# pacificclimate/VIC

Measured on AMD Instinct MI355X. Metric: cell-timesteps/s, higher is better.
Workload: dtype f64

## Files before the change

vic_amd/csrc/vic_ctx.hpp:

```cpp
#pragma once
#include <cstddef>
#include <type_traits>
#include "vic_step.hpp"

using namespace vic;

constexpr int HS_STATE = 3, HS_CLS_SHIFT = 2;

constexpr int EBC_W_POST = offsetof(SurfEBConst, delta_t) / 8, EBC_W_ALWAYS = offsetof(SurfEBConst, ice0) / 8,
              EBC_W_FROZEN = offsetof(SurfEBConst, kappa_snow) / 8, EBC_W_SNOWCOV = offsetof(SurfEBConst, LongSnowIn) / 8,
              EBC_W_INCL = offsetof(SurfEBConst, lmoist) / 8, EBC_W_EVAP = offsetof(SurfEBConst, Wdew) / 8,
              EBC_W_CANOPY = offsetof(SurfEBConst, Cs2) / 8;
constexpr int EBM_W_FEED = offsetof(SurfEBMut, deltaCC) / 8, EBM_W_IN3 = offsetof(SurfEBMut, Tsnow_surf) / 8,
              EBM_W_TSNOW = offsetof(SurfEBMut, ra_used) / 8, EBM_W_RA1 = EBM_W_TSNOW + 1, EBM_W_VV = offsetof(SurfEBMut, vv) / 8,
              EBM_W_KEEP = offsetof(SurfEBMut, Tnew2) / 8;
static_assert(offsetof(SurfEBMut, fusion) / 8 == EBM_W_IN3 - 1 && offsetof(SurfEBMut, layerevap) / 8 == EBM_W_VV + 3, "SurfEBMut layout");
constexpr size_t CW_SV = sizeof(SurfSolve) / 8, CW_EBM = sizeof(SurfEBMut) / 8, CW_EBC = EBC_W_CANOPY,
                 CW_P = sizeof(SubStep) / 8, CW_L = sizeof(SubLoop) / 8, CW_C = sizeof(StepConst) / 8;
constexpr size_t CO_SV = 0, CO_EBM = CO_SV + CW_SV, CO_EBC = CO_EBM + CW_EBM, CO_P = CO_EBC + CW_EBC, CO_L = CO_P + CW_P,
                 CO_C = CO_L + CW_L, CO_W = CO_C + CW_C;
constexpr size_t CW_W = sizeof(WCarry) / 8, CO_WM = CO_W + CW_W;
template <int NN> constexpr size_t ctx_words() { return CO_WM + sizeof(WCarryMulti<NN>) / 8; }
static_assert(sizeof(StepConstPost) <= sizeof(StepConst), "StepConstPost is parked in StepConst's words");
constexpr size_t CW_L_HEAD = offsetof(SubLoop, st_AlbedoOver) / 8;
constexpr size_t CW_SV_ITER = offsetof(SurfSolve, Tsurf) / 8;

constexpr int CTX_GROUP = 8, CTX_GROUP_B = 2;
constexpr size_t CTX_NA = sizeof(SurfSolve) / 8 + sizeof(SurfEBMut) / 8 + offsetof(SurfEBConst, Cs2) / 8;
static_assert(CTX_NA == CO_P, "region A of the context slab = what the evaluation kernel reads");
constexpr int CTXR_ITER = 0, CTXR_COMMON = 16, CTXR_CLASS = 48, CTXR_SNOW = 64, CTXR_COLD = 72, CTXR_END = 104;
struct CtxMap { unsigned char slab[CTX_NA]; int end[6]; };
constexpr int ctx_map_run(CtxMap& m, int at, size_t first, size_t last) {
  for (size_t w = first; w < last; w++) m.slab[w] = (unsigned char)at++;
  return at;
}
constexpr CtxMap ctx_make_map() {
  CtxMap m{};
  int at = ctx_map_run(m, CTXR_ITER, CO_SV, CO_SV + CW_SV_ITER);
  m.end[0] = at;
  at = ctx_map_run(m, CTXR_COMMON, CO_EBM + EBM_W_FEED, CO_EBM + EBM_W_TSNOW);
  at = ctx_map_run(m, at, CO_EBM + EBM_W_RA1, CO_EBM + EBM_W_RA1 + 1);
  at = ctx_map_run(m, at, CO_EBC, CO_EBC + EBC_W_ALWAYS);
  m.end[1] = at;
  at = ctx_map_run(m, CTXR_CLASS, CO_EBC + EBC_W_ALWAYS, CO_EBC + EBC_W_FROZEN);
  at = ctx_map_run(m, at, CO_EBC + EBC_W_INCL, CO_EBC + EBC_W_CANOPY);
  m.end[2] = at;
  at = ctx_map_run(m, CTXR_SNOW, CO_EBC + EBC_W_FROZEN, CO_EBC + EBC_W_INCL);
  m.end[3] = at;
// ... 1 lines not shown
  m.end[4] = at;
  at = ctx_map_run(m, at, CO_EBM + EBM_W_TSNOW, CO_EBM + EBM_W_TSNOW + 1);
  at = ctx_map_run(m, at, CO_EBM, CO_EBM + EBM_W_FEED);
  at = ctx_map_run(m, at, CO_EBM + EBM_W_VV, CO_EBM + CW_EBM);
  m.end[5] = at;
  return m;
}
constexpr CtxMap CTX_MAP = ctx_make_map();
constexpr bool ctx_map_is_permutation() {
  bool used[CTXR_END] = {};
  for (size_t w = 0; w < CTX_NA; w++) {
    if (CTX_MAP.slab[w] >= CTXR_END || used[CTX_MAP.slab[w]]) return false;
    used[CTX_MAP.slab[w]] = true;
  }
  int n = 0;
  for (int i = 0; i < CTXR_END; i++) n += used[i] ? 1 : 0;
  return n == (int)CTX_NA;
}
static_assert(ctx_map_is_permutation(), "parking map of region A");
static_assert(CTXR_ITER % CTX_GROUP == 0 && CTXR_COMMON % CTX_GROUP == 0 && CTXR_CLASS % CTX_GROUP == 0 && CTXR_SNOW % CTX_GROUP == 0
              && CTXR_COLD % CTX_GROUP == 0 && CTXR_END % CTX_GROUP == 0, "every range of the parking map starts on a sector boundary");
static_assert(CTX_MAP.end[0] == CTXR_COMMON && CTX_MAP.end[1] <= CTXR_CLASS && CTX_MAP.end[2] <= CTXR_SNOW && CTX_MAP.end[3] <= CTXR_COLD
              && CTX_MAP.end[4] <= CTXR_COLD + CTX_GROUP && CTX_MAP.end[5] <= CTXR_END && CTXR_END - CTX_MAP.end[5] < CTX_GROUP,
              "ranges of the parking map; the tail of SurfSolve, which every evaluation fetches, in one sector");
static_assert(CTX_MAP.end[1] - CTXR_COMMON == 31 && CTX_MAP.end[2] - CTXR_CLASS == 13,
              "the iteration's inputs: 4 sectors for every class, 2 more for frozen soil / evaporation / canopy");
constexpr size_t CTX_NA_PAD = CTXR_END;
constexpr size_t ctx_padded_words(size_t words) {
  return CTX_NA_PAD + ((words > CTX_NA ? words - CTX_NA : 0) + CTX_GROUP_B - 1) / CTX_GROUP_B * CTX_GROUP_B;
}
struct CtxRef {
  unsigned long long* p;
  int lane;
  VIC_DEV static CtxRef at(unsigned long long* base, size_t words_per_hru, size_t g) {
    return CtxRef{base + (g >> 6) * (ctx_padded_words(words_per_hru) * 64), (int)(g & 63)};
  }
  VIC_DEV unsigned long long* word(size_t W) const {
    if (W < CTX_NA) {
      const size_t S = CTX_MAP.slab[W];
      return p + (S / CTX_GROUP) * (64 * CTX_GROUP) + lane * CTX_GROUP + (S % CTX_GROUP);
    }
    const size_t V = W - CTX_NA;
    return p + CTX_NA_PAD * 64 + (V / CTX_GROUP_B) * (64 * CTX_GROUP_B) + lane * CTX_GROUP_B + (V % CTX_GROUP_B);
  }
};
template <class T>
VIC_DEV void ctx_put(const CtxRef& r, size_t word0, const T& v) {
// ... 5 lines not shown
  for (int i = 0; i < NW; i++) *r.word(word0 + i) = tmp[i];
}
template <class T>
VIC_DEV void ctx_get(const CtxRef& r, size_t word0, T& v) {
  static_assert(sizeof(T) % 8 == 0 && std::is_trivially_copyable<T>::value, "context structs are arrays of 8-byte words");
  constexpr int NW = sizeof(T) / 8;
  unsigned long long tmp[NW];
#pragma unroll
  for (int i = 0; i < NW; i++) tmp[i] = *r.word(word0 + i);
  __builtin_memcpy(&v, tmp, sizeof(T));
}

template <class T>
VIC_DEV void ctx_put_words(const CtxRef& r, size_t word0, const T& v, int first, int last) {
  constexpr int NW = sizeof(T) / 8;
#pragma unroll
  for (int i = 0; i < NW; i++)
    if (i >= first && i < last) {
      unsigned long long w;
      __builtin_memcpy(&w, reinterpret_cast<const char*>(&v) + 8 * i, 8);
      *r.word(word0 + i) = w;
    }
}
template <class T>
VIC_DEV void ctx_get_words(const CtxRef& r, size_t word0, T& v, int first, int last) {
  constexpr int NW = sizeof(T) / 8;
#pragma unroll
  for (int i = 0; i < NW; i++)
    if (i >= first && i < last) {
      const unsigned long long w = *r.word(word0 + i);
      __builtin_memcpy(reinterpret_cast<char*>(&v) + 8 * i, &w, 8);
    }
}

VIC_DEV int surf_eb_class(const SurfEBConst& c) {
  return (c.frozen_on ? EBG_FROZEN : 0) | ((c.snow_coverage > 0 && !c.INCLUDE_SNOW) ? EBG_SNOWCOV : 0) | (c.INCLUDE_SNOW ? EBG_INCL : 0)
         | (!c.SNOWING ? EBG_EVAP : 0) | ((c.VEG && !c.SNOWING) ? EBG_CANOPY : 0);
}
VIC_DEV void ebc_put(const CtxRef& cx, const SurfEBConst& c, int cls) {
  ctx_put_words(cx, CO_EBC, c, 0, EBC_W_ALWAYS);
  if (cls & EBG_FROZEN) ctx_put_words(cx, CO_EBC, c, EBC_W_ALWAYS, EBC_W_FROZEN);
  if (cls & EBG_SNOWCOV) ctx_put_words(cx, CO_EBC, c, EBC_W_FROZEN, EBC_W_SNOWCOV);
  if (cls & EBG_INCL) ctx_put_words(cx, CO_EBC, c, EBC_W_SNOWCOV, EBC_W_INCL);
  if (cls & EBG_EVAP) ctx_put_words(cx, CO_EBC, c, EBC_W_INCL, EBC_W_EVAP);
  if (cls & EBG_CANOPY) ctx_put_words(cx, CO_EBC, c, EBC_W_EVAP, EBC_W_CANOPY);
}
// ... 9 lines not shown
```

vic_amd/csrc/vic_implicit.hpp:

```cpp
#pragma once
#include "vic_profile.hpp"

namespace vic {

enum { PI_MOIST = 0, PI_ICE, PI_KAPPA, PI_CS, PIMP };

struct IArgs {
  int ncell, nhru, Nband;
  const double* pimp;
  const int* hpi;
  const double* cell_params;
  const int* hkey;
  int* fb_list;
  int* fb_count;
  int* lastexp;
  int* cursor;
};

struct ImplicitSolver {
  static constexpr int M = VIC_MID_NODES + 2;
  int n, NOFLUX, EXP_TRANS;
  double deltat, Bexp, Ts, Tb;
  double T0[M], moist[M], ice[M], kappa[M], Cs[M];
  double ice_new[M], Cs_new[M], kappa_new[M];
// ... 180 lines not shown
          const double Dp = cv.s(CP_DP);
          S.Bexp = a.EXP_TRANS ? (a.NOFLUX ? log(Dp + 1.) / (double)S.n : log(Dp + 1.) / (double)(S.n + 1)) : 0.0;
          S.Ts = S.T0[0];
          S.Tb = a.NOFLUX ? S.T0[S.n] : S.T0[S.n + 1];
          for (int q = 0; q < ImplicitSolver::M; q++) xs[q] = 0;
          S.begin(xs);
          k = 0;
          have = true;
        }
      }
    }
    if (!__any(have)) break;
    bool failed = false;
    if (have) {
      const bool conv = S.trial(xs, k);
      k++;
      if (conv) {
        const int ps = a.pslot[hru];
        double* __restrict__ rec = a.pout + (size_t)hru * pout_hru_stride(Nn) + ps * pout_stride(Nn);
        const int le = x.lastexp[hru];
        unsigned long long meta = 1ull << 32;
        if (le >= 0) {
          const double* __restrict__ src = a.pout + (size_t)hru * pout_hru_stride(Nn) + le * pout_stride(Nn);
          meta = (unsigned long long)__double_as_longlong(src[Nn]) | (1ull << 32);
          if (le != ps)
            for (int q = 0; q < (Nn + 1) / 2; q++) rec[Nn + 1 + q] = src[Nn + 1 + q];
        } else {
          int* __restrict__ cnt = reinterpret_cast<int*>(rec + Nn + 1);
          for (int q = 0; q < Nn; q++) cnt[q] = 0;
        }
        rec[0] = S.T0[0];
        for (int q = 0; q < S.n; q++) rec[q + 1] = xs[q];
        if (!a.NOFLUX) rec[Nn - 1] = S.T0[Nn - 1];
        rec[Nn] = __longlong_as_double((long long)meta);
        a.pout[(size_t)hru * pout_hru_stride(Nn) + pout_key(Nn, ps)] = S.T0[0];
        if (le >= 0) x.lastexp[hru] = ps;
        have = false;
      } else if (k >= ImplicitSolver::MAXTRIAL) {
        failed = true;
        x.lastexp[hru] = a.pslot[hru];
        have = false;
      }
    }
    list_append(x.fb_list, x.fb_count, a.cap, failed, failed ? x.hkey[hru] : 0, hru);
  }
}
```

vic_amd/csrc/vic_kernels.hpp:

```cpp
#pragma once
#include <cstddef>
#include "vic_glacier.hpp"
#include "vic_profile.hpp"
#include "vic_implicit.hpp"
#include "vic_ctx.hpp"
#include "vic_hru_io.hpp"

using namespace vic;

template <int NN, bool GLAC>
VIC_DEV int hru_prologue(const KArgs& a, int g, const HruId& id, const CellView& cv, const VegLib& vl, const Forcing& fc, const Soil3& s3,
                         HruWork<NN>& w, StepConst& C, bool node_props = true) {
  const Opt& o = a.o;
  const size_t nh = a.nhru;
  const int month = a.dmy.month;
  const int veg_idx = id.veg_idx;
  int err = 0;
  C.veg_idx = veg_idx; C.band = id.band; C.is_art_bare = id.is_art_bare ? 1 : 0;
#pragma unroll
  for (int l = 0; l < 3; l++) C.root[l] = (double)(float)a.hpd[(size_t)(HPD_ROOT0 + l) * nh + g];
  if (o.BLOWING) {
    C.sigma_slope = (double)(float)a.hpd[(size_t)HPD_SIGMA_SLOPE * nh + g]; C.lag_one = (double)(float)a.hpd[(size_t)HPD_LAG_ONE * nh + g];
    C.fetch = (double)(float)a.hpd[(size_t)HPD_FETCH * nh + g];
  } else { C.sigma_slope = 0; C.lag_one = 0; C.fetch = 0; }
// ... 179 lines not shown
    load_untouched_state<NN>(a, g, w);
    if constexpr (MULTI) {
      ctx_get(cx, CO_C, C);
      WCarryMulti<NN> km;
      ctx_get(cx, CO_WM, km);
      carry_in_multi<NN>(km, w);
    } else {
      StepConstPost q;
      ctx_get(cx, CO_C, q);
      step_const_post_in(q, P.UnderStory, C);
      C.veg_idx = id.veg_idx; C.band = id.band; C.is_art_bare = id.is_art_bare ? 1 : 0;
      C.overstory = (vl.f(id.veg_idx, VL_OVERSTORY) != 0.0) ? 1 : 0;
#pragma unroll
      for (int l = 0; l < 3; l++) C.root[l] = (double)(float)a.hpd[(size_t)(HPD_ROOT0 + l) * a.nhru + g];
    }
    {
      WCarry k;
      ctx_get(cx, CO_W, k);
      carry_in<NN>(k, w);
    }
    PROF_ADD(11, t_stage);
    PROF_T0(t_post);
    const double* __restrict__ po = a.pout + (size_t)g * pout_hru_stride(Nn) + sv.final_slot * pout_stride(Nn);
    const int* __restrict__ poc = reinterpret_cast<const int*>(po + Nn + 1);
    double Tprof[NN];
    int cntprof[NN];
    const unsigned long long flags = (unsigned long long)__double_as_longlong(po[Nn]);
#pragma unroll
    for (int n = 0; n < NN; n++) {
      Tprof[n] = (n < Nn) ? po[n] : 0.0;
      cntprof[n] = (n < Nn) ? poc[n] : 0;
    }
    using mask_t = typename NodeBound<NN>::mask_t;
    sf_sub_post<NN>(o, cv, vl, s3, fc, a.dmy, C, w, L, P, eb, sv, Tprof, cntprof,
                    (mask_t)(flags & ((1ull << NodeBound<NN>::ok_bit) - 1ull)));
    PROF_ADD(12, t_post);
    more = true;
  }
  bool pend = false;
  int key = 0;
  if ((FIRST || MULTI) && more && L.hidx < L.endhidx) {
    if constexpr (FIRST || MULTI) {
      SubStep P;
      SurfEB eb;
      SurfSolve sv;
      PROF_T0(t_pre);
      sf_sub_pre<NN>(o, cv, vl, s3, fc, a.dmy, C, w, L, P, eb, sv);
      PROF_ADD(13, t_pre);
      PROF_T0(t_put);
      ctx_put(cx, CO_SV, sv);
      ctx_put_words(cx, CO_EBM, static_cast<const SurfEBMut&>(eb), 0, EBM_W_KEEP);
      const int cls = surf_eb_class(eb);
      ebc_put(cx, eb, cls);
// ... 33 lines not shown
      if (o.IMPLICIT) {
        double* __restrict__ im = a.pimp + (size_t)g * Nn * PIMP;
#pragma unroll
        for (int n = 0; n < NN; n++)
          if (n < Nn) {
            im[n * PIMP + PI_MOIST] = w.nd.moist[n]; im[n * PIMP + PI_ICE] = (n == 0) ? eb.delta_t : w.nd.ice[n];
            im[n * PIMP + PI_KAPPA] = w.nd.kappa[n]; im[n * PIMP + PI_CS] = w.nd.Cs[n];
          }
        a.lastexp[g] = -1;
      }
      a.ts[g] = sv.x;
      a.pslot[g] = 0;
      if (o.QUICK_SOLVE) {
        int tmpNnodes = 0;
#pragma unroll
        for (int n = NN - 1; n >= 0; n--)
          if (n <= Nn - 5 && w.nd.T[n] >= 0 && w.nd.T[(n + 1 < NN) ? n + 1 : n] < 0) tmpNnodes = n + 1;
        if (tmpNnodes == 0) tmpNnodes = (w.nd.T[0] <= 0 && w.nd.T[1] >= 0) ? Nn : 3;
        else tmpNnodes += 4;
        a.jl[g] = (sv.stage == SurfSolve::ROOT_QUICK) ? tmpNnodes - 1 : (o.NOFLUX ? Nn : Nn - 1);
      }
      a.pout[(size_t)g * pout_hru_stride(Nn) + pout_key(Nn, 0)] = NAN;
      a.pout[(size_t)g * pout_hru_stride(Nn) + pout_key(Nn, 1)] = NAN;
      a.hstate[g] = 1 | (cls << HS_CLS_SHIFT);
      pend = true;
      PROF_ADD(14, t_put);
    }
  } else {
    PROF_T0(t_end);
    if (more && !sf_end<NN>(o, cv, s3, C, w, L)) err |= VICGPU_CELLERR_SOLVER;
    PROF_ADD(15, t_end);
    hru_epilogue<NN>(a, g, cv, s3, C, w, err, false);
    a.hstate[g] = 0;
  }
  list_append(a.list, a.count, a.list_cap, pend, key, g);
  PROF_ADD(0, t_stage);
  PROF_WAVE(0);
  PROF_LANE(1);
}

struct EArgs {
  Opt o;
  LaunchMap map;
  int ncell, nhru, Nn;
  const int* glist;
  int gcount;
  const double* cell_params;
// ... 6 lines not shown
  int* jl;
  int* hstate;
  int* list_next;
  int* count_next;
  int list_cap;
  const int* hkey;
  int* profile_next;
  int* pend_list_next;
  int* pend_count_next;
  int pend_cap;
  int list_thr;
  const int* pend_list_cur;
  const int* pend_prefix;
  const int* npend_cur;
  int implicit;
  const double* veglib;
  const double* forcing;
  const int* fcol;
  int ncol;
  int month;
};

constexpr int EVAL_WAVES = 2;
__global__ __launch_bounds__(64) VIC_WAVES_PER_EU(EVAL_WAVES, EVAL_WAVES) void vic_surf_eval(const EArgs a) {
  if (blockIdx.x == 0 && threadIdx.x == 0) *a.profile_next = 0;
  const int npend = *a.npend_cur;
  int g;
  if (npend <= a.list_thr) {
    if ((int)blockIdx.x * 64 >= npend) return;
    __shared__ int prefix[PEND_STRIPES + 1];
    for (int b = threadIdx.x; b < PEND_STRIPES + 1; b += 64) prefix[b] = a.pend_prefix[b];
    __syncthreads();
    const int gi = blockIdx.x * 64 + threadIdx.x;
    if (gi >= npend) return;
    int lo = 0, hi = PEND_STRIPES;
#pragma unroll
    for (int it = 0; it < 6; it++) {
      const int mid = (lo + hi) >> 1;
      const bool up = prefix[mid] <= gi;
      lo = up ? mid : lo; hi = up ? hi : mid;
    }
    g = a.pend_list_cur[(size_t)lo * a.pend_cap + (gi - prefix[lo])];
  } else {
    const int gi = a.map.index(blockIdx.x, threadIdx.x, a.gcount);
    if (gi < 0) return;
    g = a.glist ? a.glist[gi] : gi;
  }
  const int hs = a.hstate[g];
  if ((hs & HS_STATE) != 1) return;
  const int cls = hs >> HS_CLS_SHIFT;
  const size_t nh = a.nhru;
  const int c = a.hpi[(size_t)HPI_CELL * nh + g];
  const int veg_idx = a.hpi[(size_t)HPI_VEG_INDEX * nh + g];
  const int ps = a.pslot[g];
  CellView cv{a.cell_params, a.ncell, c, a.o.Nnode, a.o.Nband};
  const Soil3 s3 = load_soil3(cv);
  SurfSolve sv;
  SurfEB eb;
  const CtxRef cx = CtxRef::at(a.ctx, a.ctx_words, g);
  ctx_get(cx, CO_SV, sv);
  ebc_get(cx, eb, cls);
  const bool is_final = sv.stage == SurfSolve::FINAL;
  const int slot = sv.on_record ? sv.final_slot : ps;
  {
    SurfEBMut& m = eb;
    if (is_final) ctx_get_words(cx, CO_EBM, m, 0, EBM_W_KEEP);
    else {
      if (cls & EBG_INCL) ctx_get_words(cx, CO_EBM, m, 0, EBM_W_FEED);
      ctx_get_words(cx, CO_EBM, m, EBM_W_FEED, EBM_W_IN3);
      if (cls & EBG_SNOWCOV) ctx_get_words(cx, CO_EBM, m, EBM_W_IN3, EBM_W_TSNOW);
      if (cls & EBG_CANOPY) ctx_get_words(cx, CO_EBM, m, EBM_W_RA1, EBM_W_RA1 + 1);
    }
  }
  {
    const VegLib vl{a.veglib};
    const Forcing fc{a.forcing, nullptr, a.ncell, c, a.o.NR + 1, a.fcol[g], a.ncol};
    surf_cell_fill(eb, cv, vl, s3, fc, eb.hidx, veg_idx, a.month);
  }
  const double* __restrict__ rec = a.pout + (size_t)g * pout_hru_stride(a.Nn);
  const double* __restrict__ po = rec + slot * pout_stride(a.Nn);
  const bool ok = (((unsigned long long)__double_as_longlong(po[a.Nn])) >> record_ok_bit(node_bound(a.Nn))) & 1ull;
  if (sv.stage == SurfSolve::FINAL) sv.final_slot = slot;
  const double fx = ok ? eb.eval(a.o, s3, sv.x, po[1], po[2]) : ERROR_VAL;
  const bool was_quick = sv.stage == SurfSolve::ROOT_QUICK;
  const int stage_before = sv.stage;
  const double x_eval = sv.x;
  surf_solve_consume(a.o, sv, eb, eb, fx);
  bool at_root = false;
  if (stage_before == SurfSolve::ROOT && sv.stage == SurfSolve::FINAL && !a.implicit && !a.o.QUICK_SOLVE && !(cls & EBG_INCL) && sv.ok
      && sv.fbflag == 0 && sv.Tsurf == x_eval && fabs(fx) < 1.e30) {
    sv.final_slot = slot;
    surf_solve_consume(a.o, sv, eb, eb, fx);
    at_root = true;
  }
  if (was_quick && sv.stage != SurfSolve::ROOT_QUICK) {
    a.jl[g] = (sv.stage == SurfSolve::ROOT && a.o.NOFLUX) ? a.Nn : a.Nn - 1;
    a.pout[(size_t)g * pout_hru_stride(a.Nn) + pout_key(a.Nn, 0)] = NAN;
    a.pout[(size_t)g * pout_hru_stride(a.Nn) + pout_key(a.Nn, 1)] = NAN;
  }
  bool need_solve = sv.stage != SurfSolve::DONE;
  if (sv.stage == SurfSolve::FINAL && !a.implicit) {
    if (rec[pout_key(a.Nn, slot)] == sv.x) { sv.final_slot = slot; sv.on_record = 1; need_solve = false; }
    else if (rec[pout_key(a.Nn, slot ^ 1)] == sv.x) { sv.final_slot = slot ^ 1; sv.on_record = 1; need_solve = false; }
  }
  if (sv.stage == stage_before && (sv.stage == SurfSolve::ROOT || sv.stage == SurfSolve::ROOT_QUICK)) ctx_put_words(cx, CO_SV, sv, 0, (int)CW_SV_ITER);
  else ctx_put(cx, CO_SV, sv);
  if (sv.stage == SurfSolve::DONE) {
    const SurfEBMut& m = eb;
    if (at_root) {
      ctx_put_words(cx, CO_EBM, m, EBM_W_KEEP, (int)CW_EBM);
      ctx_put_words(cx, CO_EBM, m, EBM_W_TSNOW, EBM_W_TSNOW + 1);
      if (cls & EBG_FROZEN) ctx_put_words(cx, CO_EBM, m, EBM_W_IN3 - 1, EBM_W_IN3);
      if (cls & EBG_CANOPY) ctx_put_words(cx, CO_EBM, m, EBM_W_VV, EBM_W_VV + 6);
      else if (cls & EBG_EVAP) ctx_put_words(cx, CO_EBM, m, EBM_W_VV + 3, EBM_W_VV + 4);
    } else ctx_put(cx, CO_EBM, m);
  } else if (cls & EBG_INCL) ctx_put_words(cx, CO_EBM, static_cast<const SurfEBMut&>(eb), 0, EBM_W_FEED);
  if (sv.stage == SurfSolve::DONE) a.hstate[g] = 2;
  else if (need_solve) { a.ts[g] = sv.x; a.pslot[g] = slot ^ 1; }
  list_append(a.list_next, a.count_next, a.list_cap, need_solve, a.hkey[g], g);
  {
    const bool pend = sv.stage != SurfSolve::DONE;
    const unsigned long long m = __ballot(pend);
    if (m != 0) {
      const int lane = (int)__lane_id(), lead = __ffsll((long long)m) - 1, stripe = blockIdx.x % PEND_STRIPES;
      int base = 0;
      if (lane == lead) base = atomicAdd(a.pend_count_next + stripe * PEND_CNT_STRIDE, __popcll(m));
      base = __shfl(base, lead);
      if (pend) a.pend_list_next[(size_t)stripe * a.pend_cap + base + __popcll(m & ((1ull << lane) - 1ull))] = g;
    }
// ... 3 lines not shown
```

vic_amd/csrc/vic_pipeline.hpp:

```cpp
#pragma once
#include <hip/hip_runtime.h>
#include <stdio.h>
#include <stdlib.h>
#include <string.h>
#include <algorithm>
#include <chrono>
#include <condition_variable>
#include <memory>
#include <mutex>
#include <string>
#include <vector>
#include "vicgpu.h"
#include "vic_profile.hpp"
#include "vic_putdata.hpp"
#include "vic_host.hpp"
#include "vic_implicit.hpp"
#include "vic_ctx.hpp"
#include "vic_hru_io.hpp"
#include "vic_kernels.hpp"
#include "vic_aux_kernels.hpp"
#include "vic_records.hpp"
#include "vic_copy_cells.hpp"
#include "vic_params.hpp"
#include "vic_state_update.hpp"
// ... 52 lines not shown
  DevBuf<int> d_hstate, d_pslot, d_hkey, d_lastexp, d_jl;
  DevBuf<double> d_pimp;
  std::vector<FdChunk> chunks;
  bool put_on = false;
  int out_nrow = 0;
  OutLayout out_lay;
  DevBuf<double> d_out_data, d_out_agg, d_pb;
  DevBuf<unsigned char> d_rowagg;
};

constexpr int COPY_NKEY = 4;
constexpr int COPY_KEY_ROWS[COPY_NKEY] = {HPI_BAND, HPI_VEG_CLASS, HPI_IS_GLACIER, HPI_IS_ARTIFICIAL_BARE};

struct Tuning {
  bool node_newton = false;
  int eval_list_pct = 75;
  int nchunk = 1;
  int profile_waves_pct = 100;
  bool xcd_map = true;
  bool trace_rounds = false;
  bool trace = false;
  bool stats = false;
  int copy_stage_mb = 256;
};
static Tuning read_tuning(int node_solver, int ncell) {
  Tuning t;
  t.node_newton = node_solver == VIC_NODE_SOLVER_NEWTON;
  if (const char* ev = getenv("VICGPU_NODE_SOLVER")) t.node_newton = (strcmp(ev, "newton") == 0);
  if (const char* ev = getenv("VICGPU_EVAL_LIST_PCT")) {
    const int pct = atoi(ev);
    if (pct >= 0 && pct <= 100) t.eval_list_pct = pct;
  }
  t.nchunk = (ncell >= 20000) ? 2 : 1;
  if (const char* ev = getenv("VICGPU_CHUNKS")) t.nchunk = atoi(ev);
  if (t.nchunk < 1) t.nchunk = 1;
  if (t.nchunk > 16) t.nchunk = 16;
  if (t.nchunk > ncell) t.nchunk = ncell;
  t.profile_waves_pct = t.nchunk > 1 ? 50 : 100;
  if (const char* ev = getenv("VICGPU_PROFILE_WAVES_PCT")) {
    const int pct = atoi(ev);
    if (pct >= 5 && pct <= 100) t.profile_waves_pct = pct;
  }
  t.xcd_map = getenv("VICGPU_NO_XCD_MAP") == nullptr;
  t.trace_rounds = getenv("VICGPU_TRACE_ROUNDS") != nullptr;
  t.trace = getenv("VICGPU_TRACE") != nullptr;
  t.stats = getenv("VICGPU_STATS") != nullptr;
  if (const char* ev = getenv("VICGPU_COPY_STAGE_MB")) {
    const int mb = atoi(ev);
    if (mb >= 0 && mb <= 65536) t.copy_stage_mb = mb;
  }
  return t;
}


struct RecordsJoin {
  std::mutex m;
  std::condition_variable cv;
  std::vector<int> arrived;
  int queued = 0;
  int status = 0;
  std::string err;
  void start(int nrecords) { arrived.assign(nrecords, 0); queued = 0; status = 0; err.clear(); }
  bool arrive(int k, int nlane) { std::lock_guard<std::mutex> lk(m); return ++arrived[k] == nlane; }
  void join_queued(int k) { { std::lock_guard<std::mutex> lk(m); queued = k + 1; } cv.notify_all(); }
  int wait_queued(int k, std::string* why) {
    std::unique_lock<std::mutex> lk(m);
    cv.wait(lk, [&]() { return queued > k || status != 0; });
    if (status != 0) *why = err;
    return status;
  }
  void fail(int st, const std::string& why) {
    { std::lock_guard<std::mutex> lk(m); if (status == 0) { status = st; err = why; } }
    cv.notify_all();
// ... 251 lines not shown
  const int nsub = c->o.NF;
  for (int p = 1; p <= nsub; p++) {
    int nmax = ch->gcount;
    int npend = -1;
    int rb_list[RB_DEPTH];
    int rb_first = -1;
    for (int round = 0;; round++) {
      pa.list = ch->d_list[cur]; pa.count = cnt_list(ch->d_count, cur); pa.count_zero = cnt_list(ch->d_count, cur ^ 1);
      pa.pend_counts = cnt_list(ch->d_count, cur); pa.pend_stripes = cnt_stripes(ch->d_count, cur);
      pa.pend_stripes_zero = cnt_stripes(ch->d_count, cur ^ 1);
      if (c->o.IMPLICIT) {
        HIPCHK(ch, hipMemsetAsync(ch->d_fb_count, 0, sizeof(int) * (NBUCKET + 1), st));
        const int nblk = std::min(std::max((nmax + 63) / 64, 1), 4096);
        hipLaunchKernelGGL(vic_profile_solve_implicit, dim3(nblk), dim3(64), 0, st, pa, ia);
        HIPCHK(ch, hipGetLastError());
        pa.list = ch->d_fb_list; pa.count = ch->d_fb_count;
      }
      HIPCHK(ch, NODE_DISPATCH(Nn, launch_profile, pa, nmax, c->profile_waves, c->tune.node_newton, st));
      ea.list_next = ch->d_list[cur ^ 1]; ea.count_next = cnt_list(ch->d_count, cur ^ 1);
      ea.pend_list_next = ch->d_plist[cur ^ 1]; ea.pend_count_next = cnt_stripes(ch->d_count, cur ^ 1);
      ea.pend_list_cur = ch->d_plist[cur];
      ea.list_thr = round > 0 ? list_thr : -1;
      const bool sparse = npend >= 0 && npend <= ea.list_thr;
      hipLaunchKernelGGL(vic_surf_eval, dim3(sparse ? ((npend + 63) / 64 > 0 ? (npend + 63) / 64 : 1) : ea.map.nblocks(ch->gcount)), dim3(64), 0, st, ea);
      HIPCHK(ch, hipGetLastError());
      cur ^= 1;
      ch->rounds++;
      if (c->tune.trace_rounds) {
        int n = 0, np = 0;
        if (fd_read_count(ch, cur, &n, &np) != VICGPU_OK) return VICGPU_ERR_HIP;
        fprintf(stderr, "vicgpu rounds: chunk %d sub-step %d round %d leaves %d solves + %d evaluation-only of %d\n", (int)(ch - &c->dom.chunks[0]), p, round, n, np - n, ch->gcount);
      }
      if (round + 2 >= FREE_ROUNDS) {
        const int slot = round % RB_DEPTH;
        if (rb_first < 0) rb_first = round;
        HIPCHK(ch, hipMemcpyAsync(ch->h_count + slot * CNT_TOTAL, ch->d_count, sizeof(int) * CNT_TOTAL, hipMemcpyDeviceToHost, st));
        HIPCHK(ch, hipEventRecord(ch->readback[slot], st));
        rb_list[slot] = cur;
      }
      if (rb_first >= 0 && round - RB_LAG >= rb_first) {
        const int slot = (round - RB_LAG) % RB_DEPTH;
        HIPCHK(ch, hipEventSynchronize(ch->readback[slot]));
        const int* h = ch->h_count + slot * CNT_TOTAL;
        int n = 0;
        for (int b = 0; b < NBUCKET; b++) n += h[rb_list[slot] * CNT_LIST_STRIDE + b];
        const int np = cnt_pending(h, rb_list[slot]);
        if (np == 0) break;
// ... 307 lines not shown
```

vic_amd/csrc/vic_profile.hpp:

```cpp
#pragma once
#include "vic_surface.hpp"

namespace vic {

constexpr int NBUCKET = 2 * (VIC_MID_NODES + 2);
static_assert(NBUCKET <= 64, "one lane per work-list segment when the pending total is summed");
constexpr int PEND_STRIPES = 64, PEND_CNT_STRIDE = 32;

VIC_DEV void list_append(int* __restrict__ list, int* count, int cap, bool pred, int key, int g) {
  if (__ballot(pred) == 0) return;
  unsigned long long mine = 0;
#pragma unroll 1
  for (int k = 0; k < NBUCKET; k++) {
    const unsigned long long m = __ballot(pred && key == k);
    if (key == k) mine = m;
  }
  const int lane = (int)__lane_id();
  const int rank = __popcll(mine & ((1ull << lane) - 1ull));
  int base = 0;
  if (pred && rank == 0) base = atomicAdd(count + key, __popcll(mine));
  base = __shfl(base, pred ? __ffsll((long long)mine) - 1 : lane);
  if (pred) list[(size_t)key * cap + base + rank] = g;
}

struct PArgs {
  const double* __restrict__ pin;
  const double* __restrict__ ts;
  double* __restrict__ pout;
  const int* __restrict__ pslot;
  const int* __restrict__ list;
  const int* __restrict__ count;
  int cap;
  int* next;
  int* count_zero;
  const int* pend_counts;
  const int* pend_stripes;
  int* pend_stripes_zero;
  int* pend_prefix;
  int* pend_out;
  int Nn, NOFLUX, EXP_TRANS, TFALLBACK;
  const int* jl;
};

__host__ __device__ inline int pout_stride(int Nn) { return Nn + 1 + (Nn + 1) / 2; }
__host__ __device__ inline int pout_hru_stride(int Nn) { return 2 * pout_stride(Nn) + 2; }
__host__ __device__ inline int pout_key(int Nn, int slot) { return 2 * pout_stride(Nn) + slot; }

constexpr int LOCKSTEP_GATE = 16;

constexpr double NODE_ROOT_RANGE = SOIL_DT + Brent::MAXTRIES * Brent::TSTEP;
constexpr double NODE_NEWTON_TOL = 1.e-8;
constexpr double NODE_PREDICT_TOL2 = 1.e-7;
constexpr int NODE_PREDICT_MAXIT = 12;
constexpr double NODE_NEWTON_ACCEPT = 2.e-11;
constexpr int NODE_NEWTON_MAXIT = 200;

struct NodeK {
  double AT0, B, C, D, EI, S, G, Y, EM, EMM;
  VIC_DEV void load(const double* __restrict__ r) {
    AT0 = r[PR_AT0]; B = r[PR_B]; C = r[PR_C]; D = r[PR_D]; EI = r[PR_EI]; S = r[PR_S]; G = r[PR_G]; Y = r[PR_Y];
    EM = r[PR_EMOIST]; EMM = r[PR_EMM];
  }
  VIC_DEV double eice(double T, double& Eu, bool& curved) const {
    Eu = G * exp(Y * ln_pos(-T));
    curved = true;
    if (Eu > EMM) { Eu = EMM; curved = false; }
    double Ei = EM - Eu;
    if (Ei < 0.) { Ei = 0.; curved = false; }
    if (Ei > EMM) { Ei = EMM; curved = false; }
// ... 262 lines not shown
      PROF_WAVE(16); PROF_VOTE(17, sweeping);
#pragma unroll
      for (int j = 1; j < NN; j++) {
        if (j < jlast) {
          const double oldT = T[j];
          const double Tdn = (j == Nn - 1) ? oldT : T[(j + 1 < NN) ? j + 1 : j], Tup = T[j - 1];
          const double T0j = T0(j);
          NodeK Kj;
          if (j == NN - 1) Kj.load(a.pin + ((size_t)hru * Nn + j) * PREC);
          else {
            constexpr int q = 0;
            const int jj = (j < NN - 1) ? j : 1 + q;
            Kj.AT0 = kAT0[jj]; Kj.B = kB[jj]; Kj.C = kC[jj]; Kj.D = kD[jj]; Kj.EI = kEI[jj]; Kj.S = kS[jj]; Kj.EMM = kEMM[jj];
            Kj.G = KL(0, jj); Kj.Y = KL(1, jj); Kj.EM = KL(2, jj);
          }
          bool failed;
          double newT;
          const bool swj = sweeping && j < jl_lane;
          if (j == 1) newT = node_visit<true, NEWTON>(swj, frozen_on, EXP_TRANS, Kj, oldT, Tdn, Tup, T0j, failed);
          else newT = node_visit<false, NEWTON>(swj, frozen_on, EXP_TRANS, Kj, oldT, Tdn, Tup, T0j, failed);
          if (swj) {
            if (failed) {
              if (a.TFALLBACK) {
                int* cnt = reinterpret_cast<int*>(a.pout + (size_t)hru * pout_hru_stride(Nn) + ps * pout_stride(Nn) + Nn + 1);
                if (evcnt == 0) {
#pragma unroll
                  for (int k = 0; k < NN; k++) cnt[k] = 0;
                }
                evcnt = 1;
                cnt[j] += 1;
                newT = T0j; fbmask |= (1u << j);
              } else { ok = false; sweeping = false; }
            }
            if (sweeping) {
              T[j] = newT;
              const double diff = fabs(oldT - newT);
              if (diff > maxdiff) maxdiff = diff;
            }
          }
        }
      }
      if (sweeping) {
        if (maxdiff <= threshold) { converged = true; sweeping = false; }
        else if (it >= MAXIT) sweeping = false;
        else it++;
      }
    }
    PROF_ADD(21, t_sweep);
    PROF_T0(t_fin);
    if (have && !sweeping) {
      double T0v[NN];
      int cadd[NN];
#pragma unroll
      for (int k = 0; k < NN; k++) T0v[k] = T0(k);
      profile_finish<NN>(a.jl ? (jl_lane + 1 < Nn ? jl_lane + 1 : Nn) : Nn, a.TFALLBACK != 0, converged, ok, fbmask, T, T0v, cadd);
      double* __restrict__ rec = a.pout + (size_t)hru * pout_hru_stride(Nn) + ps * pout_stride(Nn);
      int* __restrict__ cnt = reinterpret_cast<int*>(rec + Nn + 1);
#pragma unroll
      for (int k = 0; k < NN; k++) rec[k] = T[k];
      rec[Nn] = __longlong_as_double((long long)((unsigned long long)fbmask | ((unsigned long long)(ok ? 1 : 0) << 32)));
#pragma unroll
      for (int k = 0; k < NN; k++) {
        if (evcnt == 0) cnt[k] = cadd[k];
        else cnt[k] += cadd[k];
      }
      a.pout[(size_t)hru * pout_hru_stride(Nn) + pout_key(Nn, ps)] = T0(0);
      have = false;
    }
    PROF_ADD(24, t_fin);
  }
#undef T0
#undef KL
}

constexpr int LS_WAVES = 2;
template <int NN, bool NEWTON>
__global__ __launch_bounds__(64) VIC_WAVES_PER_EU(LS_WAVES, LS_WAVES) void vic_profile_solve_lockstep(const PArgs a) {
  using mask_t = typename NodeBound<NN>::mask_t;
  constexpr bool T0_LDS = NN <= VIC_MID_NODES;
  __shared__ int bcount[NBUCKET];
  __shared__ double Tl[NN * 64];
  __shared__ double T0l[T0_LDS ? NN * 64 : 1];
  const int lane = threadIdx.x;
#define T(j) Tl[(j) * 64 + lane]
#define T0(j) (T0_LDS ? T0l[(T0_LDS ? (j) : 0) * 64 + lane] : ((j) == 0 ? T0s : blk[(j) * PREC + PR_T0]))
  for (int b = lane; b < NBUCKET; b += 64) bcount[b] = a.count[b];
  if (blockIdx.x == 0) {
    for (int b = lane; b < NBUCKET; b += 64) a.count_zero[b] = 0;
    int v = (lane < NBUCKET) ? a.pend_counts[lane] : 0;
#pragma unroll
    for (int off = 32; off >= 1; off >>= 1) v += __shfl(v, lane ^ off);
    pend_pack(a, lane, v);
  }
  __syncthreads();
  int n = 0;
#pragma unroll
  for (int b = 0; b < NBUCKET; b++) n += bcount[b];
  if ((int)blockIdx.x * 64 >= n) return;

  const int Nn = node_count<NN>(a.Nn);
  const int jlast = a.NOFLUX ? Nn : Nn - 1;
  const int MAXIT = 1000;
  const double threshold = 1.e-2;
  const bool EXP_TRANS = a.EXP_TRANS != 0;

#define LS_REC() (a.pout + (size_t)hru * pout_hru_stride(Nn) + ps * pout_stride(Nn))
#define LS_CNT(j) (reinterpret_cast<int*>(LS_REC() + Nn + 1)[j])
  bool have = false, sweeping = false, converged = false, ok = true, frozen_on = false;
  int hru = 0, ps = 0, it = 1, jl_lane = 0;
  mask_t fbmask = 0;
  const double* __restrict__ blk = a.pin;
  double T0s = 0;
  bool more = true;
  while (true) {
    const unsigned long long idle = __ballot(!have);
    if (more && (__popcll(idle) >= LOCKSTEP_GATE || idle == ~0ull)) {
      const int nidle = __popcll(idle), leader = __ffsll((long long)idle) - 1;
      int base = 0;
      if (lane == leader) base = atomicAdd(a.next, nidle);
      base = __builtin_amdgcn_readlane(base, leader);
      if (base + nidle >= n) more = false;
      const int slot = base + __popcll(idle & ((1ull << lane) - 1ull));
      if (!have && slot < n) {
        hru = profile_pick(a, bcount, slot);
        blk = a.pin + (size_t)hru * Nn * PREC;
        ps = a.pslot[hru];
        jl_lane = a.jl ? a.jl[hru] : jlast;
        frozen_on = blk[PR_AT0] != 0.0;
        const double Ts = a.ts[hru];
#pragma unroll
// ... 51 lines not shown
    }
    if (have && !sweeping) {
      const int nq = a.jl ? (jl_lane + 1 < Nn ? jl_lane + 1 : Nn) : Nn;
      if (ok && a.TFALLBACK) {
#pragma unroll 1
        for (int k = 1; k < nq - 1; k++) {
          const double Tk = T(k), Tm = T(k - 1), Tp = T(k + 1), Lk = T0(k), Lm = T0(k - 1), Lp = T0(k + 1);
          if (Lm - Lk > 0 && Lp - Tk > 0 && (Tm - Tk) - (Lm - Lk) > 0 && (Tp - Tk) - (Lp - Lk) > 0) {
            T(k) = 0.5 * (Tm + Tp);
            fbmask |= (mask_t(1) << k);
            LS_CNT(k) += 1;
          }
        }
      }
      if (ok && !converged) {
        if (a.TFALLBACK) {
#pragma unroll 1
          for (int k = 0; k < nq; k++) { T(k) = T0(k); LS_CNT(k) += 1; }
          fbmask |= node_mask_below<NN>(nq);
        } else ok = false;
      }
      double* __restrict__ rec = LS_REC();
#pragma unroll 1
      for (int k = 0; k < Nn; k++) rec[k] = T(k);
      rec[Nn] = profile_flag_word<NN>(fbmask, ok);
      a.pout[(size_t)hru * pout_hru_stride(Nn) + pout_key(Nn, ps)] = T0(0);
      have = false;
    }
  }
}
#undef T
#undef T0
#undef LS_REC
#undef LS_CNT

}
```

Before: 4.066 million.

## Sector-align profile records and keep solver stage bits in hstate to trim eval traffic

Profile output records are reordered so the flag word and the first temperatures sit in the first 8-word sector, and record and per-HRU strides are rounded to sector multiples. The surface-evaluation kernel gains a template variant that reads only the iteration words of SurfSolve. The stage, on-record flag and final slot are carried in hstate bits instead of the slab tail, and the kernel writes back only the words that changed. This aims to cut memory sectors touched per evaluation. In exchange it adds padding, more per-word branches, and a fallback full-tail path kept for QUICK_SOLVE.

New measurement: 4.129 million, median of 3. Within noise of the previous version (+1.6%).

```diff
diff --git a/vic_amd/csrc/vic_ctx.hpp b/vic_amd/csrc/vic_ctx.hpp
--- a/vic_amd/csrc/vic_ctx.hpp
+++ b/vic_amd/csrc/vic_ctx.hpp
@@ -5,7 +5,10 @@
 
 using namespace vic;
 
-constexpr int HS_STATE = 3, HS_CLS_SHIFT = 2;
+constexpr int HS_STATE = 3, HS_CLS_SHIFT = 2, HS_CLS_MASK = 31;
+constexpr int HS_FINAL = 1 << 7, HS_ON_RECORD = 1 << 8, HS_FINAL_SLOT_SHIFT = 9, HS_FINAL_SLOT = 1 << HS_FINAL_SLOT_SHIFT;
+static_assert((EBG_FROZEN | EBG_SNOWCOV | EBG_INCL | EBG_EVAP | EBG_CANOPY) == HS_CLS_MASK && (HS_CLS_MASK << HS_CLS_SHIFT) < HS_FINAL,
+              "hstate: state, class, stage bits do not overlap");
 
 constexpr int EBC_W_POST = offsetof(SurfEBConst, delta_t) / 8, EBC_W_ALWAYS = offsetof(SurfEBConst, ice0) / 8,
               EBC_W_FROZEN = offsetof(SurfEBConst, kappa_snow) / 8, EBC_W_SNOWCOV = offsetof(SurfEBConst, LongSnowIn) / 8,
@@ -24,6 +27,14 @@
 static_assert(sizeof(StepConstPost) <= sizeof(StepConst), "StepConstPost is parked in StepConst's words");
 constexpr size_t CW_L_HEAD = offsetof(SubLoop, st_AlbedoOver) / 8;
 constexpr size_t CW_SV_ITER = offsetof(SurfSolve, Tsurf) / 8;
+constexpr size_t CW_SV_TSURF = offsetof(SurfSolve, Tsurf) / 8, CW_SV_ERROR = offsetof(SurfSolve, error) / 8,
+                 CW_SV_STAGE = offsetof(SurfSolve, stage) / 8, CW_SV_OK = offsetof(SurfSolve, ok) / 8,
+                 CW_SV_SLOT = offsetof(SurfSolve, final_slot) / 8;
+static_assert(offsetof(SurfSolve, stage) % 8 == 0 && offsetof(SurfSolve, fbflag) == offsetof(SurfSolve, stage) + 4
+              && offsetof(SurfSolve, fbcount) % 8 == 0 && offsetof(SurfSolve, ok) == offsetof(SurfSolve, fbcount) + 4
+              && offsetof(SurfSolve, final_slot) % 8 == 0 && offsetof(SurfSolve, on_record) == offsetof(SurfSolve, final_slot) + 4
+              && CW_SV_SLOT + 1 == CW_SV && CW_SV_OK == CW_SV_STAGE + 1 && CW_SV_SLOT == CW_SV_OK + 1,
+              "SurfSolve tail: {stage, fbflag} {fbcount, ok} {final_slot, on_record}, low half first");
 
 constexpr int CTX_GROUP = 8, CTX_GROUP_B = 2;
 constexpr size_t CTX_NA = sizeof(SurfSolve) / 8 + sizeof(SurfEBMut) / 8 + offsetof(SurfEBConst, Cs2) / 8;
@@ -71,7 +82,7 @@
               && CTXR_COLD % CTX_GROUP == 0 && CTXR_END % CTX_GROUP == 0, "every range of the parking map starts on a sector boundary");
 static_assert(CTX_MAP.end[0] == CTXR_COMMON && CTX_MAP.end[1] <= CTXR_CLASS && CTX_MAP.end[2] <= CTXR_SNOW && CTX_MAP.end[3] <= CTXR_COLD
               && CTX_MAP.end[4] <= CTXR_COLD + CTX_GROUP && CTX_MAP.end[5] <= CTXR_END && CTXR_END - CTX_MAP.end[5] < CTX_GROUP,
-              "ranges of the parking map; the tail of SurfSolve, which every evaluation fetches, in one sector");
+              "ranges of the parking map; the tail of SurfSolve in one sector");
 static_assert(CTX_MAP.end[1] - CTXR_COMMON == 31 && CTX_MAP.end[2] - CTXR_CLASS == 13,
               "the iteration's inputs: 4 sectors for every class, 2 more for frozen soil / evaporation / canopy");
 constexpr size_t CTX_NA_PAD = CTXR_END;
@@ -123,6 +134,7 @@
       *r.word(word0 + i) = w;
     }
 }
+VIC_DEV void ctx_put_half(const CtxRef& r, size_t word, int half, int v) { reinterpret_cast<int*>(r.word(word))[half] = v; }
 template <class T>
 VIC_DEV void ctx_get_words(const CtxRef& r, size_t word0, T& v, int first, int last) {
   constexpr int NW = sizeof(T) / 8;
diff --git a/vic_amd/csrc/vic_implicit.hpp b/vic_amd/csrc/vic_implicit.hpp
--- a/vic_amd/csrc/vic_implicit.hpp
+++ b/vic_amd/csrc/vic_implicit.hpp
@@ -226,17 +226,17 @@
         unsigned long long meta = 1ull << 32;
         if (le >= 0) {
           const double* __restrict__ src = a.pout + (size_t)hru * pout_hru_stride(Nn) + le * pout_stride(Nn);
-          meta = (unsigned long long)__double_as_longlong(src[Nn]) | (1ull << 32);
+          meta = (unsigned long long)__double_as_longlong(src[pout_flag()]) | (1ull << 32);
           if (le != ps)
-            for (int q = 0; q < (Nn + 1) / 2; q++) rec[Nn + 1 + q] = src[Nn + 1 + q];
+            for (int q = 0; q < (Nn + 1) / 2; q++) rec[pout_cnt(Nn) + q] = src[pout_cnt(Nn) + q];
         } else {
-          int* __restrict__ cnt = reinterpret_cast<int*>(rec + Nn + 1);
+          int* __restrict__ cnt = reinterpret_cast<int*>(rec + pout_cnt(Nn));
           for (int q = 0; q < Nn; q++) cnt[q] = 0;
         }
-        rec[0] = S.T0[0];
-        for (int q = 0; q < S.n; q++) rec[q + 1] = xs[q];
-        if (!a.NOFLUX) rec[Nn - 1] = S.T0[Nn - 1];
-        rec[Nn] = __longlong_as_double((long long)meta);
+        rec[pout_T(0)] = S.T0[0];
+        for (int q = 0; q < S.n; q++) rec[pout_T(q + 1)] = xs[q];
+        if (!a.NOFLUX) rec[pout_T(Nn - 1)] = S.T0[Nn - 1];
+        rec[pout_flag()] = __longlong_as_double((long long)meta);
         a.pout[(size_t)hru * pout_hru_stride(Nn) + pout_key(Nn, ps)] = S.T0[0];
         if (le >= 0) x.lastexp[hru] = ps;
         have = false;
diff --git a/vic_amd/csrc/vic_kernels.hpp b/vic_amd/csrc/vic_kernels.hpp
--- a/vic_amd/csrc/vic_kernels.hpp
+++ b/vic_amd/csrc/vic_kernels.hpp
@@ -225,13 +225,13 @@
     PROF_ADD(11, t_stage);
     PROF_T0(t_post);
     const double* __restrict__ po = a.pout + (size_t)g * pout_hru_stride(Nn) + sv.final_slot * pout_stride(Nn);
-    const int* __restrict__ poc = reinterpret_cast<const int*>(po + Nn + 1);
+    const int* __restrict__ poc = reinterpret_cast<const int*>(po + pout_cnt(Nn));
     double Tprof[NN];
     int cntprof[NN];
-    const unsigned long long flags = (unsigned long long)__double_as_longlong(po[Nn]);
+    const unsigned long long flags = (unsigned long long)__double_as_longlong(po[pout_flag()]);
 #pragma unroll
     for (int n = 0; n < NN; n++) {
-      Tprof[n] = (n < Nn) ? po[n] : 0.0;
+      Tprof[n] = (n < Nn) ? po[pout_T(n)] : 0.0;
       cntprof[n] = (n < Nn) ? poc[n] : 0;
     }
     using mask_t = typename NodeBound<NN>::mask_t;
@@ -311,7 +311,7 @@
       }
       a.pout[(size_t)g * pout_hru_stride(Nn) + pout_key(Nn, 0)] = NAN;
       a.pout[(size_t)g * pout_hru_stride(Nn) + pout_key(Nn, 1)] = NAN;
-      a.hstate[g] = 1 | (cls << HS_CLS_SHIFT);
+      a.hstate[g] = 1 | (cls << HS_CLS_SHIFT) | (sv.stage == SurfSolve::FINAL ? HS_FINAL : 0);
       pend = true;
       PROF_ADD(14, t_put);
     }
@@ -364,6 +364,7 @@
 };
 
 constexpr int EVAL_WAVES = 2;
+template <bool FULL_TAIL>
 __global__ __launch_bounds__(64) VIC_WAVES_PER_EU(EVAL_WAVES, EVAL_WAVES) void vic_surf_eval(const EArgs a) {
   if (blockIdx.x == 0 && threadIdx.x == 0) *a.profile_next = 0;
   const int npend = *a.npend_cur;
@@ -390,7 +391,7 @@
   }
   const int hs = a.hstate[g];
   if ((hs & HS_STATE) != 1) return;
-  const int cls = hs >> HS_CLS_SHIFT;
+  const int cls = (hs >> HS_CLS_SHIFT) & HS_CLS_MASK;
   const size_t nh = a.nhru;
   const int c = a.hpi[(size_t)HPI_CELL * nh + g];
   const int veg_idx = a.hpi[(size_t)HPI_VEG_INDEX * nh + g];
@@ -400,8 +401,14 @@
   SurfSolve sv;
   SurfEB eb;
   const CtxRef cx = CtxRef::at(a.ctx, a.ctx_words, g);
-  ctx_get(cx, CO_SV, sv);
+  if constexpr (FULL_TAIL) ctx_get(cx, CO_SV, sv);
+  else ctx_get_words(cx, CO_SV, sv, 0, (int)CW_SV_ITER);
   ebc_get(cx, eb, cls);
+  if constexpr (!FULL_TAIL) {
+    sv.stage = (hs & HS_FINAL) ? SurfSolve::FINAL : SurfSolve::ROOT;
+    sv.on_record = (hs & HS_ON_RECORD) ? 1 : 0; sv.final_slot = (hs >> HS_FINAL_SLOT_SHIFT) & 1;
+    sv.Ts_old = eb.Ts_old; sv.snow_surf_temp = 0; sv.Tsurf = 0; sv.error = 0; sv.fbflag = 0; sv.fbcount = 0; sv.ok = 1;
+  }
   const bool is_final = sv.stage == SurfSolve::FINAL;
   const int slot = sv.on_record ? sv.final_slot : ps;
   {
@@ -421,15 +428,16 @@
   }
   const double* __restrict__ rec = a.pout + (size_t)g * pout_hru_stride(a.Nn);
   const double* __restrict__ po = rec + slot * pout_stride(a.Nn);
-  const bool ok = (((unsigned long long)__double_as_longlong(po[a.Nn])) >> record_ok_bit(node_bound(a.Nn))) & 1ull;
+  const bool ok = (((unsigned long long)__double_as_longlong(po[pout_flag()])) >> record_ok_bit(node_bound(a.Nn))) & 1ull;
   if (sv.stage == SurfSolve::FINAL) sv.final_slot = slot;
-  const double fx = ok ? eb.eval(a.o, s3, sv.x, po[1], po[2]) : ERROR_VAL;
-  const bool was_quick = sv.stage == SurfSolve::ROOT_QUICK;
+  const double fx = ok ? eb.eval(a.o, s3, sv.x, po[pout_T(1)], po[pout_T(2)]) : ERROR_VAL;
+  const bool quick_solve = FULL_TAIL && a.o.QUICK_SOLVE;
+  const bool was_quick = FULL_TAIL && sv.stage == SurfSolve::ROOT_QUICK;
   const int stage_before = sv.stage;
   const double x_eval = sv.x;
   surf_solve_consume(a.o, sv, eb, eb, fx);
   bool at_root = false;
-  if (stage_before == SurfSolve::ROOT && sv.stage == SurfSolve::FINAL && !a.implicit && !a.o.QUICK_SOLVE && !(cls & EBG_INCL) && sv.ok
+  if (stage_before == SurfSolve::ROOT && sv.stage == SurfSolve::FINAL && !a.implicit && !quick_solve && !(cls & EBG_INCL) && sv.ok
       && sv.fbflag == 0 && sv.Tsurf == x_eval && fabs(fx) < 1.e30) {
     sv.final_slot = slot;
     surf_solve_consume(a.o, sv, eb, eb, fx);
@@ -445,8 +453,23 @@
     if (rec[pout_key(a.Nn, slot)] == sv.x) { sv.final_slot = slot; sv.on_record = 1; need_solve = false; }
     else if (rec[pout_key(a.Nn, slot ^ 1)] == sv.x) { sv.final_slot = slot ^ 1; sv.on_record = 1; need_solve = false; }
   }
-  if (sv.stage == stage_before && (sv.stage == SurfSolve::ROOT || sv.stage == SurfSolve::ROOT_QUICK)) ctx_put_words(cx, CO_SV, sv, 0, (int)CW_SV_ITER);
-  else ctx_put(cx, CO_SV, sv);
+  if constexpr (FULL_TAIL) {
+    if (sv.stage == stage_before && (sv.stage == SurfSolve::ROOT || sv.stage == SurfSolve::ROOT_QUICK)) ctx_put_words(cx, CO_SV, sv, 0, (int)CW_SV_ITER);
+    else ctx_put(cx, CO_SV, sv);
+  } else if (is_final) {
+    ctx_put_words(cx, CO_SV, sv, (int)CW_SV_ERROR, (int)CW_SV_ERROR + 1);
+    ctx_put_words(cx, CO_SV, sv, (int)CW_SV_SLOT, (int)CW_SV_SLOT + 1);
+    ctx_put_half(cx, CO_SV + CW_SV_STAGE, 0, sv.stage);
+    if (!sv.ok) ctx_put_half(cx, CO_SV + CW_SV_OK, 1, 0);
+  } else {
+    ctx_put_words(cx, CO_SV, sv, 0, (int)CW_SV_ITER);
+    if (sv.stage != stage_before) {
+      ctx_put_words(cx, CO_SV, sv, (int)CW_SV_TSURF, (int)CW_SV_TSURF + 1);
+      ctx_put_words(cx, CO_SV, sv, (int)CW_SV_ERROR, (int)CW_SV);
+      if (sv.stage != SurfSolve::DONE)
+        a.hstate[g] = hs | HS_FINAL | (sv.on_record ? HS_ON_RECORD : 0) | (sv.final_slot << HS_FINAL_SLOT_SHIFT);
+    }
+  }
   if (sv.stage == SurfSolve::DONE) {
     const SurfEBMut& m = eb;
     if (at_root) {
diff --git a/vic_amd/csrc/vic_pipeline.hpp b/vic_amd/csrc/vic_pipeline.hpp
--- a/vic_amd/csrc/vic_pipeline.hpp
+++ b/vic_amd/csrc/vic_pipeline.hpp
@@ -98,6 +98,7 @@
   bool trace = false;
   bool stats = false;
   int copy_stage_mb = 256;
+  bool eval_full_tail = false;
 };
 static Tuning read_tuning(int node_solver, int ncell) {
   Tuning t;
@@ -125,6 +126,7 @@
     const int mb = atoi(ev);
     if (mb >= 0 && mb <= 65536) t.copy_stage_mb = mb;
   }
+  t.eval_full_tail = getenv("VICGPU_EVAL_FULL_TAIL") != nullptr;
   return t;
 }
 
@@ -422,7 +424,9 @@
       ea.pend_list_cur = ch->d_plist[cur];
       ea.list_thr = round > 0 ? list_thr : -1;
       const bool sparse = npend >= 0 && npend <= ea.list_thr;
-      hipLaunchKernelGGL(vic_surf_eval, dim3(sparse ? ((npend + 63) / 64 > 0 ? (npend + 63) / 64 : 1) : ea.map.nblocks(ch->gcount)), dim3(64), 0, st, ea);
+      const dim3 egrid(sparse ? ((npend + 63) / 64 > 0 ? (npend + 63) / 64 : 1) : ea.map.nblocks(ch->gcount));
+      if (c->o.QUICK_SOLVE || c->tune.eval_full_tail) hipLaunchKernelGGL(vic_surf_eval<true>, egrid, dim3(64), 0, st, ea);
+      else hipLaunchKernelGGL(vic_surf_eval<false>, egrid, dim3(64), 0, st, ea);
       HIPCHK(ch, hipGetLastError());
       cur ^= 1;
       ch->rounds++;
diff --git a/vic_amd/csrc/vic_profile.hpp b/vic_amd/csrc/vic_profile.hpp
--- a/vic_amd/csrc/vic_profile.hpp
+++ b/vic_amd/csrc/vic_profile.hpp
@@ -42,9 +42,16 @@
   const int* jl;
 };
 
-__host__ __device__ inline int pout_stride(int Nn) { return Nn + 1 + (Nn + 1) / 2; }
-__host__ __device__ inline int pout_hru_stride(int Nn) { return 2 * pout_stride(Nn) + 2; }
-__host__ __device__ inline int pout_key(int Nn, int slot) { return 2 * pout_stride(Nn) + slot; }
+constexpr int POUT_SECTOR = 8;
+__host__ __device__ constexpr int pout_round(int words) { return (words + POUT_SECTOR - 1) / POUT_SECTOR * POUT_SECTOR; }
+__host__ __device__ constexpr int pout_flag() { return 0; }
+__host__ __device__ constexpr int pout_T(int n) { return 1 + n; }
+__host__ __device__ constexpr int pout_cnt(int Nn) { return 1 + Nn; }
+__host__ __device__ constexpr int pout_stride(int Nn) { return pout_round(1 + Nn + (Nn + 1) / 2); }
+__host__ __device__ constexpr int pout_hru_stride(int Nn) { return pout_round(2 * pout_stride(Nn) + 2); }
+__host__ __device__ constexpr int pout_key(int Nn, int slot) { return 2 * pout_stride(Nn) + slot; }
+static_assert(pout_stride(10) == 16 && pout_hru_stride(10) == 40 && pout_T(2) < POUT_SECTOR && pout_stride(VIC_MAX_NODES) % POUT_SECTOR == 0,
+              "profile records: flag word, T1 and T2 in the first sector of a sector-aligned record");
 
 constexpr int LOCKSTEP_GATE = 16;
 
@@ -353,7 +360,7 @@
           if (swj) {
             if (failed) {
               if (a.TFALLBACK) {
-                int* cnt = reinterpret_cast<int*>(a.pout + (size_t)hru * pout_hru_stride(Nn) + ps * pout_stride(Nn) + Nn + 1);
+                int* cnt = reinterpret_cast<int*>(a.pout + (size_t)hru * pout_hru_stride(Nn) + ps * pout_stride(Nn) + pout_cnt(Nn));
                 if (evcnt == 0) {
 #pragma unroll
                   for (int k = 0; k < NN; k++) cnt[k] = 0;
@@ -386,10 +393,10 @@
       for (int k = 0; k < NN; k++) T0v[k] = T0(k);
       profile_finish<NN>(a.jl ? (jl_lane + 1 < Nn ? jl_lane + 1 : Nn) : Nn, a.TFALLBACK != 0, converged, ok, fbmask, T, T0v, cadd);
       double* __restrict__ rec = a.pout + (size_t)hru * pout_hru_stride(Nn) + ps * pout_stride(Nn);
-      int* __restrict__ cnt = reinterpret_cast<int*>(rec + Nn + 1);
-#pragma unroll
-      for (int k = 0; k < NN; k++) rec[k] = T[k];
-      rec[Nn] = __longlong_as_double((long long)((unsigned long long)fbmask | ((unsigned long long)(ok ? 1 : 0) << 32)));
+      int* __restrict__ cnt = reinterpret_cast<int*>(rec + pout_cnt(Nn));
+      rec[pout_flag()] = __longlong_as_double((long long)((unsigned long long)fbmask | ((unsigned long long)(ok ? 1 : 0) << 32)));
+#pragma unroll
+      for (int k = 0; k < NN; k++) rec[pout_T(k)] = T[k];
 #pragma unroll
       for (int k = 0; k < NN; k++) {
         if (evcnt == 0) cnt[k] = cadd[k];
@@ -436,7 +443,7 @@
   const bool EXP_TRANS = a.EXP_TRANS != 0;
 
 #define LS_REC() (a.pout + (size_t)hru * pout_hru_stride(Nn) + ps * pout_stride(Nn))
-#define LS_CNT(j) (reinterpret_cast<int*>(LS_REC() + Nn + 1)[j])
+#define LS_CNT(j) (reinterpret_cast<int*>(LS_REC() + pout_cnt(Nn))[j])
   bool have = false, sweeping = false, converged = false, ok = true, frozen_on = false;
   int hru = 0, ps = 0, it = 1, jl_lane = 0;
   mask_t fbmask = 0;
@@ -534,8 +541,8 @@
       }
       double* __restrict__ rec = LS_REC();
 #pragma unroll 1
-      for (int k = 0; k < Nn; k++) rec[k] = T(k);
-      rec[Nn] = profile_flag_word<NN>(fbmask, ok);
+      for (int k = 0; k < Nn; k++) rec[pout_T(k)] = T(k);
+      rec[pout_flag()] = profile_flag_word<NN>(fbmask, ok);
       a.pout[(size_t)hru * pout_hru_stride(Nn) + pout_key(Nn, ps)] = T0(0);
       have = false;
     }
```
